# elucideye/acf

Measured on AMD Instinct MI355X. Metric: detector FPS @1080p, 8 scales/octave, FACE80 model, higher is better.
Workload: dtype f32

## Files before the change

### acf_amd/csrc/acf_hip.hip

```cpp
#include "kernels.hip.h"

#include <algorithm>
#include <cmath>
#include <cstdio>
#include <cstring>
#include <mutex>
#include <string>
#include <type_traits>
#include <vector>

using namespace acfhip;

namespace
{

struct DevBuf
{
    void* p = nullptr;
    size_t bytes = 0;
};

struct ResampleTiling
{
    int rows = 0, cols = 0, xo = 0, tile_y = 0, tile_x = 0;
// ... 108 lines not shown
    int tiles = 0, tileRows = 0, tileCols = 0;
    int maxCells = 0, maxBlocks = 0;
    float* d_tmp = nullptr;
    float* d_pyr = nullptr;
};

struct Options
{
    int taps = 0;
    int arith = 0;
    int profile = 0;
    int fusedSmooth = 1;
    int fusedGrad = 1;
    int fusedTri = 1;
    int sharedDevice = 0;
    int tilePersist = 1;
    int cascadeTiles = 1;
    int rankCells = 1;
    int scaleStreams = 1;
    int cascadeTurns = 0;
    int fusedLevels = 1;
    int smoothSegments = 0;
    int smoothWarm = 64, smoothForceRedo = 0;
    int levelSegments = 0;
    int levelWarm = 32;
    int countRepairs = 0;
    int keepPyramid = 1;
};

struct acf_hip_ctx
{
    int device = 0;
    hipStream_t stream = nullptr;
    bool ownStream = false;
    std::vector<hipStream_t> side;
    std::vector<acf_hip_ctx*> kids;
    int nStreams = 1, kidChunk = 0;
    hipEvent_t evFork = nullptr;
    std::vector<hipEvent_t> evJoin;
    mutable std::string err;
    bool hasModel = false, hasPlan = false;
    Options opt;
    bool x86Owned = false;
    uint32_t* d_x86 = nullptr;
    int numCus = 256;
    size_t ldsPerCu = size_t(160) * 1024;
    bool ranksValid = false;
    bool floatPyramid = true;
    std::vector<hipEvent_t> evPool;
    std::vector<const char*> evName;
    size_t evUsed = 0;
    std::vector<hipStream_t> evStream;
    std::vector<hipEvent_t> evScale;
    hipEvent_t evTurn[2] = { nullptr, nullptr };

    acf_hip_params p{};
    std::vector<uint32_t> fids, child;
    std::vector<float> thrs, hs;
    LdcfStage ldcf;

    Plan plan;
    bool autoLambdas = false;
    double* d_planeSums = nullptr;
    std::vector<double> h_lambdas;
    int maxBatch = 0, maxHits = 0, lastBatch = 0;
    bool pyramidValid = false, detectValid = false;

    std::vector<void*> allocs;
    float* d_lTable = nullptr;
    float* d_acos = nullptr;
    std::vector<RealScale> real;
    std::vector<ResampleDesc> h_descs;
    int nImgDescs = 0, nApproxDescs = 0;
    ResampleDesc* d_descs = nullptr;
    int32_t* d_it = nullptr;
    float* d_ft = nullptr;
    SmoothJob* d_realJobs = nullptr;
    SmoothJob* d_finalJobs = nullptr;
    LevelJob* d_levelJobs = nullptr;
    float* d_dump = nullptr;
    LevelJob* d_levelJobsRaw = nullptr;
    struct LevelGroup
    {
        int R, mode, first, count;
        double cost;
        int lane;
    };
    std::vector<LevelGroup> levelGroups, levelGroupsRaw;
    int nAllJobs = 0, nAllJobsRaw = 0;
    bool fusedOk = false;
    PadJob* d_padJobs = nullptr;
    PadJob* d_padJobsR = nullptr;
    bool levelsEmitRank = false;
    float *d_specState = nullptr, *d_trueState = nullptr;
    bool countersZeroed = false;
    int32_t* d_redo = nullptr;
    size_t redoInts = 0, lvRedoInts = 0;
    float *d_lvSpec = nullptr, *d_lvTrue = nullptr;
    int32_t* d_lvRedo = nullptr;
    int levelSegFrames = 0, levelSegCap = 0, levelHMax = 0;
    int useGraph = 0;
    struct GraphSlot
    {
        hipGraphExec_t exec = nullptr;
        const float* frames = nullptr;
        int n = 0;
// ... 46 lines not shown
    {
        int64_t chromaOff = 0, frameStride = 0;
    } yuv;
    uint8_t* d_yuvRgb = nullptr;
    size_t yuvRgbBytes = 0;
};

static inline bool rankCellsOn(const acf_hip_ctx* c, const CascState& cs)
{
    return cs.tilesR.ok && c->opt.rankCells;
}

#define HIPCHK(ctx, call)                                                                                  \
    do                                                                                                     \
    {                                                                                                      \
        hipError_t e_ = (call);                                                                            \
        if (e_ != hipSuccess)                                                                              \
        {                                                                                                  \
            (ctx)->err = std::string(#call) + ": " + hipGetErrorString(e_);                               \
            return ACF_HIP_E_HIP;                                                                          \
        }                                                                                                  \
    } while (0)

#define LAUNCHCHK(ctx, what)                                                                               \
    do                                                                                                     \
    {                                                                                                      \
        hipError_t e_ = hipGetLastError();                                                                 \
        if (e_ != hipSuccess)                                                                              \
        {                                                                                                  \
            (ctx)->err = std::string("launch ") + what + ": " + hipGetErrorString(e_);                    \
            return ACF_HIP_E_HIP;                                                                          \
        }                                                                                                  \
    } while (0)

namespace
{

enum : uint32_t
{
    FB_TRIY_UNFUSED = 1u << 0,
    FB_MOU_PLAIN = 1u << 1,
    FB_RESAMPLE_NO_STRIP = 1u << 2,
    FB_RESAMPLE_NO_PAIR = 1u << 3,
    FB_RESAMPLE_NO_UP = 1u << 4,
    FB_RESAMPLE_GENERIC = 1u << 5,
    FB_LEVEL_GROUPS = 1u << 6,
    FB_LDCF_UNFUSED = 1u << 7,
    FB_NO_DEDUP = 1u << 8,
    FB_NO_TAIL_CODES = 1u << 9,
    FB_TAIL3 = 1u << 10,
    FB_TILED_STAGED = 1u << 11,
    FB_TILED_POOLED1 = 1u << 12,
    FB_YUV_UNFUSED = 1u << 13,
};
uint32_t fallbackMask()
{
    static const uint32_t mask = [] {
        static const struct { const char* name; uint32_t bit; } kNames[] = {
            { "triy_unfused", FB_TRIY_UNFUSED }, { "mou_plain", FB_MOU_PLAIN }, { "resample_no_strip", FB_RESAMPLE_NO_STRIP },
            { "resample_no_pair", FB_RESAMPLE_NO_PAIR }, { "resample_no_up", FB_RESAMPLE_NO_UP }, { "resample_generic", FB_RESAMPLE_GENERIC },
            { "level_groups", FB_LEVEL_GROUPS }, { "ldcf_unfused", FB_LDCF_UNFUSED }, { "no_dedup", FB_NO_DEDUP }, { "no_tail_codes", FB_NO_TAIL_CODES },
            { "tail3", FB_TAIL3 }, { "tiled_staged", FB_TILED_STAGED }, { "tiled_pooled1", FB_TILED_POOLED1 },
            { "yuv_unfused", FB_YUV_UNFUSED } };
        uint32_t m = 0;
        const char* e = getenv("ACF_HIP_FORCE_FALLBACK");
        std::string s = e ? e : "";
        size_t i = 0;
        while (i < s.size())
        {
            size_t j = s.find(',', i);
            j = j == std::string::npos ? s.size() : j;
            const std::string tok = s.substr(i, j - i);
            bool known = tok.empty();
            for (const auto& n : kNames)
            {
                if (tok == n.name)
                {
                    m |= n.bit;
                    known = true;
                }
            }
            if (!known)
            {
                fprintf(stderr, "acf_hip: ACF_HIP_FORCE_FALLBACK: unknown name '%s'\n", tok.c_str());
                abort();
            }
            i = j + 1;
        }
        return m;
    }();
    return mask;
}
inline bool fallbackForced(uint32_t which)
{
    return (fallbackMask() & which) != 0;
}

int fail(const acf_hip_ctx* c, int code, const std::string& msg)
{
    c->err = msg;
    return code;
}

int needCtx(const acf_hip_ctx* c)
{
    return c ? ACF_HIP_OK : ACF_HIP_E_INVALID;
}
int needPlan(const acf_hip_ctx* c, const char* who, const char* hint = "")
{
    return !c ? ACF_HIP_E_INVALID : c->hasPlan ? ACF_HIP_OK : fail(c, ACF_HIP_E_NOPLAN, std::string(who) + ": plan first" + hint);
}
int needPlanRead(const acf_hip_ctx* c, const char* who)
{
    return c ? needPlan(c, who) : ACF_HIP_E_NOPLAN;
}
int needModel(const acf_hip_ctx* c, const char* who)
// ... 614 lines not shown
    {
        return ACF_HIP_OK;
    }
    std::lock_guard<std::mutex> lk(g_turnMu);
    HIPCHK(c, hipEventRecord(c->evTurn[which], c->stream));
    g_turnLast[chain][c->device] = c->evTurn[which];
    return ACF_HIP_OK;
}
void cascTurnForget(acf_hip_ctx* c)
{
    std::lock_guard<std::mutex> lk(g_turnMu);
    for (int w = 0; w < 2; w++)
    {
        if (c->evTurn[w])
        {
            for (int ch = 0; ch < 2; ch++)
            {
                if (c->device >= 0 && c->device < 64 && g_turnLast[ch][c->device] == c->evTurn[w])
                {
                    g_turnLast[ch][c->device] = nullptr;
                }
            }
            (void)hipEventDestroy(c->evTurn[w]);
            c->evTurn[w] = nullptr;
        }
    }
}
}

extern "C" {


int acf_hip_abi_version(void)
{
    return ACF_HIP_ABI_VERSION;
}

constexpr int ACF_SIDE_STREAMS = 6;
constexpr int LEVEL_MAX_R_REAL = 9;
static void ensureSide(acf_hip_ctx* c)
{
    while (int(c->side.size()) < std::min<int>(ACF_SIDE_STREAMS, int(c->evJoin.size())))
    {
        hipStream_t st;
        if (hipStreamCreateWithFlags(&st, hipStreamNonBlocking) != hipSuccess)
        {
            (void)hipGetLastError();
            break;
        }
        c->side.push_back(st);
    }
}

int acf_hip_create(int device, void* stream, acf_hip_ctx** out)
{
    if (!out)
    {
        return ACF_HIP_E_INVALID;
    }
    *out = nullptr;
    int n = 0;
    if (hipGetDeviceCount(&n) != hipSuccess || n <= 0 || device < 0 || device >= n)
    {
        return ACF_HIP_E_NODEVICE;
    }
    if (hipSetDevice(device) != hipSuccess)
    {
        return ACF_HIP_E_NODEVICE;
    }
    acf_hip_ctx* c = new (std::nothrow) acf_hip_ctx();
    if (!c)
    {
        return ACF_HIP_E_HIP;
    }
    c->device = device;
    {
        hipDeviceProp_t prop;
        if (hipGetDeviceProperties(&prop, device) == hipSuccess)
        {
            c->numCus = prop.multiProcessorCount > 0 ? prop.multiProcessorCount : c->numCus;
            c->ldsPerCu = prop.maxSharedMemoryPerMultiProcessor > 0 ? size_t(prop.maxSharedMemoryPerMultiProcessor) : c->ldsPerCu;
        }
    }
    if (stream)
    {
        c->stream = reinterpret_cast<hipStream_t>(stream);
    }
    else
    {
        if (hipStreamCreateWithFlags(&c->stream, hipStreamNonBlocking) != hipSuccess)
        {
            delete c;
            return ACF_HIP_E_HIP;
        }
        c->ownStream = true;
    }
    for (int i = 0; i < ACF_SIDE_STREAMS; i++)
    {
        hipEvent_t ev;
        if (hipEventCreateWithFlags(&ev, hipEventDisableTiming) == hipSuccess)
        {
            c->evJoin.push_back(ev);
        }
    }
    (void)hipEventCreateWithFlags(&c->evFork, hipEventDisableTiming);
    *out = c;
// ... 38 lines not shown
            if (!synced)
            {
                (void)hipSetDevice(c->device);
                (void)hipStreamSynchronize(c->stream);
                synced = true;
            }
            (void)hipGraphExecDestroy(g.exec);
        }
        g = acf_hip_ctx::GraphSlot();
    }
    c->graphNext = 0;
    c->plainRuns = 0;
}

int acf_hip_destroy(acf_hip_ctx* c)
{
    dropGraph(c);
    if (c)
    {
        for (acf_hip_ctx* k : c->kids)
        {
            (void)acf_hip_destroy(k);
        }
        c->kids.clear();
    }
    if (!c)
    {
        return ACF_HIP_E_INVALID;
    }
    (void)hipSetDevice(c->device);
    (void)hipStreamSynchronize(c->stream);
    (void)acf_hip_stream_close(c);
    cascTurnForget(c);
    freeAll(c);
    if (c->d_x86 && c->x86Owned)
    {
        (void)hipFree(c->d_x86);
    }
    for (hipEvent_t e : c->evPool)
    {
        (void)hipEventDestroy(e);
    }
    for (hipStream_t st : c->side)
    {
        (void)hipStreamDestroy(st);
    }
    for (hipEvent_t e : c->evJoin)
    {
        (void)hipEventDestroy(e);
    }
    if (c->evFork)
    {
        (void)hipEventDestroy(c->evFork);
    }
    for (hipEvent_t e : c->evScale)
    {
        (void)hipEventDestroy(e);
    }
    if (c->ownStream)
    {
        (void)hipStreamDestroy(c->stream);
    }
    delete c;
    return ACF_HIP_OK;
}

const char* acf_hip_last_error(const acf_hip_ctx* c)
{
    return c ? c->err.c_str() : "null context";
}

struct OptionKey
{
    const char* key;
    int Options::*field;
    bool nonzero;
    bool (*refuse)(const acf_hip_ctx*, int);
    const char* why;
    void (*after)(acf_hip_ctx*, int);
};

static bool negative(const acf_hip_ctx*, int v)
{
    return v < 0;
}

static const char* const LEVEL_RANGE = "option: level_warm a positive multiple of 4, level_segments >= 0";
static const char* const SMOOTH_RANGE = "option: smooth_segments >= 0, smooth_warm a multiple of 16";

static const OptionKey OPTION_KEYS[] = {
    { "graph", nullptr, false, nullptr, nullptr, [](acf_hip_ctx* c, int v) { c->useGraph = v; c->graphBroken = 0; } },
    { "streams", nullptr, false, [](const acf_hip_ctx*, int v) { return v < 1 || v > 6; }, "streams: 1..6",
        [](acf_hip_ctx* c, int v) { c->nStreams = v; } },
    { "taps", &Options::taps, true },
    { "arith", &Options::arith, true, [](const acf_hip_ctx* c, int v) { return v != 0 && !c->d_x86; },
        "arith: install a CPU's tables first (acf_hip_set_x86_tables)" },
    { "profile", &Options::profile, true, nullptr, nullptr, [](acf_hip_ctx* c, int) { c->evUsed = 0; } },
    { "fused_levels", &Options::fusedLevels, false },
    { "fused_smooth", &Options::fusedSmooth, true },
    { "fused_grad", &Options::fusedGrad, false },
    { "fused_tri", &Options::fusedTri, false },
    { "shared_device", &Options::sharedDevice, true },
    { "cascade_tiles", &Options::cascadeTiles, true },
    { "rank_cells", &Options::rankCells, true, nullptr, nullptr, [](acf_hip_ctx* c, int) { c->detectValid = false; } },
    { "tile_persist", &Options::tilePersist, false },
    { "cascade_turns", &Options::cascadeTurns, false },
// ... 1147 lines not shown
```

### acf_amd/csrc/kernels_channels.hip.h

```cpp
#pragma once

namespace acfhip
{

struct SmoothVecArgs
{
    const float* in;
    float* sm;
    float* half;
    float* chns;
    int64_t in_fs, in_ps, sm_fs, sm_ps, half_fs, half_ps, chns_fs, cells;
    int32_t h, w, plane0;
    float p, rkHalf, rq_y;
    float* dump;
    int32_t segW, warm, nSeg, nPlanes;
    int32_t segStride;
    float* specState;
    float* trueState;
    int32_t* redo;
    int32_t skipZ;
    float* gM;
    float* gO;
    const float* acos;
    int64_t mo_fs;
// ... 454 lines not shown
    {
        smooth_vec_body<true, HALF, true>(a, lds, z);
    }
    else
    {
        smooth_vec_body<false, HALF, true>(a, lds, z);
    }
}

template <bool HALF, bool ARITH = false>
__global__ void __launch_bounds__(64 * SV_MAXW) k_smooth_grad(SmoothVecArgs a, uint32_t fullMask)
{
    extern __shared__ float lds[];
    const int z = a.plane0;
    if (a.redo)
    {
        if (a.redo[int64_t(blockIdx.z) * a.nPlanes + z] == 0)
        {
            return;
        }
        __syncthreads();
        if (threadIdx.x == 0)
        {
            a.redo[int64_t(blockIdx.z) * a.nPlanes + z] = 0;
        }
    }
    float* acosL = lds + 2 * SV_MAXW * 2 * SV_K * 4;
    for (int i = threadIdx.x; i < GM_ACOS_N; i += blockDim.x)
    {
        acosL[i] = a.acos[i];
    }
    uint2* x86G = reinterpret_cast<uint2*>(acosL + GM_ACOS_N);
    float x86K = 0.f;
    if (ARITH)
    {
        const uint2* gsrc = reinterpret_cast<const uint2*>(a.x86 + X86_TABLE_N);
        for (int i = threadIdx.x; i < X86_GM_N; i += blockDim.x)
        {
            x86G[i] = gsrc[i];
        }
        x86K = __uint_as_float(a.x86[X86_TABLE_N + 2 * X86_GM_N]);
    }
    __syncthreads();
    if ((fullMask >> z) & 1u)
    {
        smooth_vec_body<true, HALF, true, true, false, ARITH>(a, lds, z, acosL + 10010, x86G, x86K);
    }
    else
    {
        smooth_vec_body<false, HALF, true, true, false, ARITH>(a, lds, z, acosL + 10010, x86G, x86K);
    }
}

template <bool HALF, bool ARITH = false>
__global__ void __launch_bounds__(512) k_smooth_grad_tri(SmoothVecArgs a, uint32_t fullMask)
{
    extern __shared__ float lds[];
    const int z = a.plane0;
    float* acosL = lds + 2 * SV_MAXW * 2 * SV_K * 4;
    for (int i = threadIdx.x; i < GM_ACOS_N; i += blockDim.x)
    {
        acosL[i] = a.acos[i];
    }
    uint2* x86G = reinterpret_cast<uint2*>(acosL + GM_ACOS_N);
    float x86K = 0.f;
    if (ARITH)
    {
        const uint2* gsrc = reinterpret_cast<const uint2*>(a.x86 + X86_TABLE_N);
        for (int i = threadIdx.x; i < X86_GM_N; i += blockDim.x)
        {
            x86G[i] = gsrc[i];
        }
        x86K = __uint_as_float(a.x86[X86_TABLE_N + 2 * X86_GM_N]);
    }
    __syncthreads();
    if ((fullMask >> z) & 1u)
    {
        smooth_vec_body<true, HALF, true, true, true, ARITH>(a, lds, z, acosL + 10010, x86G, x86K);
    }
    else
    {
        smooth_vec_body<false, HALF, true, true, true, ARITH>(a, lds, z, acosL + 10010, x86G, x86K);
    }
}

__global__ void __launch_bounds__(256) k_smooth_verify(const float* __restrict__ spec, const float* __restrict__ tru, int h, int segStride, int nPlanes,
    int32_t* __restrict__ redo, int force, int nSeg, int zG, int nSegG)
{
    const int64_t plane = int64_t(blockIdx.z) * nPlanes + blockIdx.y;
    const int s = 1 + blockIdx.x;
    if (s >= (int(blockIdx.y) == zG ? nSegG : nSeg))
    {
        return;
    }
    const uint32_t* a = reinterpret_cast<const uint32_t*>(spec) + (plane * segStride + s) * int64_t(h);
    const uint32_t* b = reinterpret_cast<const uint32_t*>(tru) + (plane * segStride + s) * int64_t(h);
    bool bad = force != 0;
    for (int y = threadIdx.x; y < h; y += 256)
    {
        bad = bad || (a[y] != b[y]);
    }
    if (bad)
    {
        redo[plane] = 1;
    }
}

struct SumJob
{
    int64_t off;
    int32_t cells;
    int32_t pad_;
};

__global__ void __launch_bounds__(256) k_plane_sums(const float* __restrict__ chns, int64_t chns_fs, SumJob j0, SumJob j1, int nPlanes, double* __restrict__ out)
{
    __shared__ double part[256];
    const int z = blockIdx.x, sel = blockIdx.y;
    const int64_t f = blockIdx.z;
    const SumJob J = sel ? j1 : j0;
    const float* __restrict__ src = chns + f * chns_fs + J.off + int64_t(z) * J.cells;
    double acc = 0.0;
    for (int i = threadIdx.x; i < J.cells; i += 256)
    {
        acc += double(src[i]);
    }
    part[threadIdx.x] = acc;
    __syncthreads();
    for (int s = 128; s >= 1; s >>= 1)
    {
        if (int(threadIdx.x) < s)
        {
            part[threadIdx.x] += part[threadIdx.x + s];
        }
        __syncthreads();
// ... 1231 lines not shown
```

### acf_amd/csrc/pyramid_run.hip.h

```cpp
#pragma once

namespace
{
struct ScalePlan
{
    bool fuseSm = false;
    bool halfNext = false;
    uint32_t fullMask = 0;
    bool wantGrad = false;
    bool triXFused = false;
    bool fuseCells = false;
    bool blocked = false;
    ChnsArgs a{};
    int nt = 0, warm = 0;
    int nSeg = 1, segW = 0;
    int nSegG = 1, segWG = 0;
    int segStride = 1;
    size_t ldsB = 0, ldsG = 0;
};

using SmoothVecKernel = void (*)(SmoothVecArgs, uint32_t);
using GradMagVecKernel = void (*)(const float*, float*, float*, const float*, int, int, int, int64_t, int64_t, int, int, const uint32_t*);
using LevelAllKernel = void (*)(const float*, float*, float*, const LevelJob*, const ResampleDesc*, const int32_t*, const float*, int, int64_t, int64_t, float,
    float*, int, LevelRankArgs, LevelSegArgs);
using LevelKernel = void (*)(const float*, float*, float*, const LevelJob*, const ResampleDesc*, const int32_t*, const float*, int, int64_t, int64_t, float,
    float*, int);

enum LevelsPath
{
    LV_FUSED,
    LV_WAVE_SMOOTH,
    LV_SMOOTH_JOBS,
    LV_COPY
};
struct LevelsCall
{
    LevelsPath path = LV_COPY;
    int nLF = 0;
    bool approxFirst = false;
    bool pad = false;
    float pS = 0.f;
    int64_t copyElems = 0;
    const LevelJob* jobs = nullptr;
    const std::vector<acf_hip_ctx::LevelGroup>* groups = nullptr;
    int nAll = 0;
    size_t nSide = 0;
    bool rawOut = false;
    bool emitRank = false, emitF32 = true;
    LevelRankArgs ra{};
    LevelSegArgs lsa{};
    size_t ldsL = 0;
    LevelAllKernel allKernel = nullptr;
    bool lvTurns = false;
    int lvChain = 1;
};

static SmoothVecKernel smoothGradKernel(bool tri, bool half, bool x86)
{
    if (!x86)
    {
        if (!tri)
        {
            return half ? k_smooth_grad<true, false> : k_smooth_grad<false, false>;
        }
        return half ? k_smooth_grad_tri<true, false> : k_smooth_grad_tri<false, false>;
    }
    if (!tri)
    {
        return half ? k_smooth_grad<true, true> : k_smooth_grad<false, true>;
    }
    return half ? k_smooth_grad_tri<true, true> : k_smooth_grad_tri<false, true>;
}

static SmoothVecKernel smoothVecKernel(bool half)
{
    return half ? k_smooth_vec<true> : k_smooth_vec<false>;
}

static GradMagVecKernel gradMagVecKernel(bool blocked, bool x86)
{
    if (blocked)
    {
        return x86 ? k_grad_mag_vec<true, true> : k_grad_mag_vec<true, false>;
    }
    return x86 ? k_grad_mag_vec<false, true> : k_grad_mag_vec<false, false>;
}

static LevelAllKernel levelAllKernel(bool f32, bool rank, bool segmented)
{
    if (f32 && rank)
    {
        return segmented ? k_level_all<LO_F32 | LO_RANK, 1> : k_level_all<LO_F32 | LO_RANK, 0>;
    }
    if (rank)
    {
        return segmented ? k_level_all<LO_RANK, 1> : k_level_all<LO_RANK, 0>;
    }
    return segmented ? k_level_all<LO_F32, 1> : k_level_all<LO_F32, 0>;
}

static LevelKernel levelKernel(int R, int mode)
{
#define LEVEL_R(RR)                                 \
    switch (mode)                                   \
    {                                               \
        case LM_REAL: return k_level<RR, LM_REAL>;  \
        case LM_DD: return k_level<RR, LM_DD>;      \
        default: return k_level<RR, LM_UU>;         \
    }
    switch (R)
    {
        case 1: LEVEL_R(1)
        case 2: LEVEL_R(2)
        case 3: LEVEL_R(3)
        case 4: LEVEL_R(4)
        case 5: LEVEL_R(5)
        case 6: LEVEL_R(6)
        case 7: LEVEL_R(7)
        case 8: LEVEL_R(8)
        default:
            return R == LEVEL_MAX_R_REAL && mode == LM_REAL ? k_level<9, LM_REAL> : nullptr;
    }
#undef LEVEL_R
}

static int countRepairs(acf_hip_ctx* c, hipStream_t st, const int32_t* d_flags, size_t n, int slot)
{
    if (!c->opt.countRepairs)
    {
        return ACF_HIP_OK;
    }
    std::vector<int32_t> fl(n);
    HIPCHK(c, hipMemcpyAsync(fl.data(), d_flags, n * 4, hipMemcpyDeviceToHost, st));
    HIPCHK(c, hipStreamSynchronize(st));
    c->repairs[slot] += int64_t(n);
    for (int32_t v : fl)
    {
        c->repairs[slot + 1] += v != 0;
    }
    return ACF_HIP_OK;
}

struct PyramidRun
{
    acf_hip_ctx* const c;
    const acf_hip_params& p;
    const Plan& pl;
    const int nF;
    const int H, W, d, d_in, shrink;
    const int64_t np0;
    const float* frames;
    const float* cur = nullptr;
    int64_t cur_fs = 0;
    int curH = 0, curW = 0;
    float pColor = 0.f;
    std::vector<int> srcIdx;
    std::vector<char> halfDone, pairDone;
    bool scalePar = false;
    hipStream_t st;
    LevelsCall lv;
    PackedSrc reduced{}, converted{};

    PyramidRun(acf_hip_ctx* ctx, const float* frames_, int nF_)
        : c(ctx), p(ctx->p), pl(ctx->plan), nF(nF_), H(pl.H), W(pl.W), d(pl.d), d_in(pl.d_in), shrink(ctx->p.shrink), np0(int64_t(pl.H) * pl.W), frames(frames_),
          st(ctx->stream)
    {
    }

    int ingest(const PackedSrc* u8, bool& ingestConverted);
    int colour(bool ingestConverted);
    int prepareScales();
    int realScale(size_t k);
    int imageResample(size_t k, const float*& img, int64_t& img_fs);
    ScalePlan planScale(size_t k, const float* img, int64_t img_fs);
    int smoothImage(size_t k, const float* img, int64_t img_fs, const ScalePlan& sp);
    int gradientChannels(size_t k, const ScalePlan& sp);
    int joinScales();
    int planLevels(int nLF);
    int levels(int f0, int nLF);
    int launchLevels(const LevelsCall& lc, int f0);
    int launchLevelAll(const LevelsCall& lc, int f0);
    int launchLevelGroups(const LevelsCall& lc, int f0);
    int padLevels(const LevelsCall& lc, int f0);
    int levelsWithImageLambdas();
};

int PyramidRun::ingest(const PackedSrc* u8, bool& ingestConverted)
{
    int rc;
    if (d_in == 5)
    {
        return fail(c, ACF_HIP_E_INVALID, "pyramid_u8: a plan for five input planes (image + M, O) takes float frames");
    }
    const int inRows = c->rz.on ? c->rz.rows : H, inCols = c->rz.on ? c->rz.cols : W;
    const bool fusedYuv = u8 && pixIsYuv(u8->pix) && !c->rz.on && !fallbackForced(FB_YUV_UNFUSED);
    if (u8 && pixIsYuv(u8->pix) && !fusedYuv)
    {
        U8Geom g;
        if (const char* bad = u8Geom(u8->pix, inRows, inCols, u8->rowStride, c->yuv.chromaOff, c->yuv.frameStride, g))
        {
            return fail(c, ACF_HIP_E_INVALID, std::string("pyramid_u8: ") + bad);
        }
        if (!u8PlanesOk(g, d_in))
        {
            return fail(c, ACF_HIP_E_INVALID, "pyramid_u8: the plan's input planes (d) must be 3 for NV12 / NV21");
        }
        const size_t need = size_t(c->maxBatch) * inRows * inCols * 3;
        if (c->yuvRgbBytes < need)
        {
            HIPCHK(c, hipStreamSynchronize(c->stream));
            devRelease(c, c->d_yuvRgb);
            c->yuvRgbBytes = 0;
            if ((rc = devAlloc(c, &c->d_yuvRgb, need)))
            {
                return rc;
            }
            c->yuvRgbBytes = need;
        }
        if ((rc = launchYuvToRgb(c, yuvSrc(u8->frames, u8->pix, inRows, inCols, g), nF, c->d_yuvRgb)))
        {
            return rc;
        }
        converted = PackedSrc{ c->d_yuvRgb, ACF_HIP_PIX_RGB, 0 };
        u8 = &converted;
    }
    if (u8 && c->rz.on)
    {
        U8Geom g;
// ... 69 lines not shown
        int curIdx = -1;
        for (size_t k = 0; k < c->real.size(); k++)
        {
            srcIdx[k] = curIdx;
            if (c->real[k].adoptAsI)
            {
                curIdx = int(k);
            }
        }
    }
    if (c->opt.scaleStreams && c->real.size() > 1 && !c->opt.taps)
    {
        ensureSide(c);
    }
    const size_t nSideS = c->side.size();
    scalePar = c->opt.scaleStreams && c->real.size() > 1 && nSideS >= c->real.size() - 1 && c->evJoin.size() >= nSideS && !c->opt.taps;
    while (scalePar && c->evScale.size() < c->real.size())
    {
        hipEvent_t e;
        HIPCHK(c, hipEventCreateWithFlags(&e, hipEventDisableTiming));
        c->evScale.push_back(e);
    }
    return ACF_HIP_OK;
}

int PyramidRun::realScale(size_t k)
{
    int rc;
    RealScale& rs = c->real[k];
    const int64_t np = int64_t(rs.h) * rs.w;
    if (scalePar)
    {
        if (k > 0)
        {
            prof(c, st, "(end)");
        }
        st = k == 0 ? c->stream : c->side[k - 1];
        if (k > 0)
        {
            HIPCHK(c, hipStreamWaitEvent(st, c->evScale[k - 1], 0));
        }
    }
    const float* img = cur;
    int64_t img_fs = cur_fs;
    if (rs.resampled && (rc = imageResample(k, img, img_fs)))
    {
        return rc;
    }
    const ScalePlan sp = planScale(k, img, img_fs);
    if ((rc = smoothImage(k, img, img_fs, sp)))
    {
        return rc;
    }
    if (scalePar)
    {
        HIPCHK(c, hipEventRecord(c->evScale[k], st));
    }
    if (rs.adoptAsI)
    {
        cur = rs.sm;
        cur_fs = int64_t(d) * np;
        curH = rs.h;
        curW = rs.w;
    }
    return gradientChannels(k, sp);
}

int PyramidRun::imageResample(size_t k, const float*& img, int64_t& img_fs)
{
    RealScale& rs = c->real[k];
    const int64_t np = int64_t(rs.h) * rs.w;
    if (rs.src_h != curH || rs.src_w != curW)
    {
        return fail(c, ACF_HIP_E_INVALID, "pyramid: internal plan mismatch");
    }
    if (c->h_descs[rs.descIndex].src_frame_stride != cur_fs)
    {
        return fail(c, ACF_HIP_E_INVALID, "pyramid: internal frame-stride mismatch");
    }
    prof(c, st, "k_resample(image)");
    const ResampleDesc& hd = c->h_descs[rs.descIndex];
    const bool exactHalf = hd.xmode == RS_EXACT && hd.ymode == RS_EXACT && hd.xk == 2 && hd.yk == 2 && hd.ha % 4 == 0 && hd.hb % 2 == 0 &&
        hd.src_frame_stride % 4 == 0 && hd.dst_frame_stride % 2 == 0 && hd.src_off % 4 == 0 && hd.dst_off % 2 == 0 &&
        (uintptr_t(cur) & 15) == 0 && (uintptr_t(rs.img) & 7) == 0;
    if (halfDone[k] || pairDone[k])
    {
    }
    else if (rs.strip.ok && !exactHalf && !resampleGenericOnly() && (uintptr_t(cur) & 15) == 0)
    {
        const bool pair = rs.stripPair.ok && k + 1 < c->real.size() && srcIdx[k + 1] == srcIdx[k] && !c->opt.taps && !scalePar;
        if (pair)
        {
            pairDone[k + 1] = 1;
        }
        launchStrip(c, st, pair ? rs.stripPair : rs.strip, c->d_descs, rs.descIndex, pair ? c->real[k + 1].descIndex : -1, hd.nplanes, cur, rs.img,
            pair ? c->real[k + 1].img : nullptr, c->d_it, c->d_ft, nF);
    }
    else if (exactHalf)
    {
        const int64_t items = int64_t(hd.hb / 2) * hd.wb * hd.nplanes;
        hipLaunchKernelGGL(k_resample_half, dim3(cdiv(items, 256), 1, nF), dim3(256), 0, st, cur, rs.img,
            (const ResampleDesc*)(c->d_descs + rs.descIndex));
    }
    else if (resampleUpOk(hd) && !resampleGenericOnly() && (uintptr_t(rs.img) & 15) == 0)
    {
        const int nw = hd.nplanes * cdiv(hd.hb, 256) * cdiv(hd.wb, RSU_XC);
        hipLaunchKernelGGL(k_resample_up, dim3(cdiv(nw, 4), 1, nF), dim3(256), 0, st, cur, rs.img,
            (const ResampleDesc*)(c->d_descs + rs.descIndex), (const int32_t*)c->d_it, (const float*)c->d_ft);
    }
    else
    {
        const int xt = int64_t(resampleBlocks(hd)) * nF < 4096 ? 2 : RS_XT;
        hipLaunchKernelGGL(k_resample, dim3(resampleBlocks(hd, xt), 1, nF), dim3(64, 4), 0, st, cur, rs.img,
            (const ResampleDesc*)(c->d_descs + rs.descIndex), (const int32_t*)c->d_it, (const float*)c->d_ft, xt);
    }
    LAUNCHCHK(c, "k_resample(image)");
    img = rs.img;
    img_fs = int64_t(d) * np;
// ... 9 lines not shown
    ScalePlan sp;
    sp.fuseSm = p.colorSmooth > 0 && p.colorEnabled && !c->opt.taps && c->opt.fusedSmooth && shrink == 4 && rs.h % 4 == 0 && rs.w % 4 == 0 && rs.w >= 16 &&
        rs.h / 4 <= SV_MAXW * SV_OWN && img_fs % 4 == 0 && np % 4 == 0 && (uintptr_t(img) & 15) == 0;
    ChnsArgs& a = sp.a;
    a.sm = rs.sm;
    a.M = rs.M;
    a.S = rs.S;
    a.O = rs.O;
    a.Mn = c->opt.taps ? rs.Mn : nullptr;
    a.chns = c->d_chns + pl.raw_off[rs.level];
    a.sm_fs = int64_t(d) * np;
    a.m_fs = np;
    a.chns_fs = pl.raw_floats;
    a.h = rs.h;
    a.w = rs.w;
    a.d = d;
    a.colorEnabled = p.colorEnabled;
    a.colorDone = sp.fuseSm ? 1 : 0;
    a.magEnabled = p.gradMagEnabled;
    a.histEnabled = p.gradHistEnabled;
    a.nOrients = p.nOrients;
    a.doNorm = p.normRad != 0;
    a.full = p.full;
    a.hardBin = p.softBin < 0;
    a.normConst = float(p.normConst);
    a.rq_y = shrinkGainY(shrink);
    const bool gradVec = rs.h % 4 == 0 && np % 4 == 0;
    sp.fuseCells = shrink == 4 && !c->opt.taps;
    sp.blocked = grad && p.normRad && !moWithImage &&
        triPlan(rs.M, rs.U, rs.h, rs.w, p.normRad, np, sp.fuseCells ? &a : nullptr, rs.uFloats, rs.moFloats, gradVec).blocked;
    if (!sp.fuseSm)
    {
        return sp;
    }
    sp.halfNext = k + 1 < c->real.size() && srcIdx[k + 1] == int(k) && c->real[k + 1].resampled && [&] {
        const ResampleDesc& nd = c->h_descs[c->real[k + 1].descIndex];
        return nd.xmode == RS_EXACT && nd.ymode == RS_EXACT && nd.xk == 2 && nd.yk == 2 && nd.ha == rs.h && nd.wa == rs.w;
    }();
    bool needFullAll = false;
    for (size_t m = k + 1; m < c->real.size(); m++)
    {
        if (srcIdx[m] == int(k) && !(m == k + 1 && sp.halfNext))
        {
            needFullAll = true;
        }
    }
    sp.nt = cdiv(rs.h / 4, SV_OWN) * 64;
    const int64_t gradMinPx = int64_t(1) << 20;
    const int gradMinF = 16;
    sp.wantGrad = grad && gradVec && !moWithImage && (c->opt.fusedGrad >= 2 || (c->opt.fusedGrad == 1 && np >= gradMinPx && nF >= gradMinF));
    const int triMinF = 64;
    sp.triXFused = sp.wantGrad && sp.blocked && p.normRad == 5 && rs.w >= 48 && sp.nt <= 512 &&
        (c->opt.fusedTri >= 2 || (c->opt.fusedTri == 1 && c->opt.sharedDevice && nF >= triMinF));
    for (int z = 0; z < d; z++)
    {
        if (needFullAll || (grad && z == p.colorChn && !sp.wantGrad))
        {
            sp.fullMask |= 1u << z;
        }
    }
    sp.warm = std::max(16, c->opt.smoothWarm);
    auto segmentsFor = [&](int planesOf, int& segW_) {
        int n = c->opt.smoothSegments;
        if (n == 0 && c->opt.sharedDevice && nF >= 64)
        {
            n = 1;
        }
        if (n == 0)
        {
            const int64_t waves = int64_t(std::max(planesOf, 1)) * nF * (sp.nt / 64);
            n = int(std::min<int64_t>((6 * 1024 + waves - 1) / waves, rs.w / (4 * sp.warm)));
        }
        n = std::max(1, std::min(n, std::min(c->segCap, rs.w / 16)));
        segW_ = cdiv(cdiv(rs.w, n), 16) * 16;
        return cdiv(rs.w, segW_);
    };
    if (!sp.wantGrad)
    {
        sp.nSeg = sp.nSegG = segmentsFor(d, sp.segW);
        sp.segWG = sp.segW;
    }
    else
    {
        if (sp.triXFused)
        {
            sp.nSegG = 1;
            sp.segWG = cdiv(rs.w, 16) * 16;
        }
        else
        {
            sp.nSegG = segmentsFor(1, sp.segWG);
        }
        sp.nSeg = sp.nSegG;
        sp.segW = sp.segWG;
        if (d > 1)
        {
            sp.nSeg = segmentsFor(d - 1, sp.segW);
        }
    }
    sp.segStride = std::max(sp.nSeg, sp.nSegG);
    sp.ldsB = size_t(2) * SV_MAXW * 2 * SV_K * 4 * sizeof(float);
    sp.ldsG = sp.ldsB + size_t(GM_ACOS_N) * sizeof(float) + (c->opt.arith ? size_t(X86_GM_N) * sizeof(uint2) : 0);
    return sp;
}

int PyramidRun::smoothImage(size_t k, const float* img, int64_t img_fs, const ScalePlan& sp)
{
    int rc;
    RealScale& rs = c->real[k];
    const int64_t np = int64_t(rs.h) * rs.w;
    if (!sp.fuseSm)
    {
        if (p.colorSmooth > 0)
        {
            return launchSmooth(c, st, img, rs.sm, c->d_realJobs + k, 1, d, rs.h, img_fs, int64_t(d) * np, nF, pColor, true);
        }
        hipLaunchKernelGGL(k_copy_planes, dim3(cdiv(np * d, 256), 1, nF), dim3(256), 0, st, img, rs.sm, (const SmoothJob*)(c->d_realJobs + k), img_fs,
            int64_t(d) * np);
        LAUNCHCHK(c, "k_copy_planes");
        return ACF_HIP_OK;
    }
    SmoothVecArgs sa{};
    sa.in = img;
    sa.in_fs = img_fs;
    sa.in_ps = np;
    sa.sm = rs.sm;
    sa.sm_fs = int64_t(d) * np;
    sa.sm_ps = np;
    sa.chns = c->d_chns + pl.raw_off[rs.level];
    sa.chns_fs = pl.raw_floats;
    sa.cells = int64_t(rs.h / 4) * (rs.w / 4);
    sa.h = rs.h;
    sa.w = rs.w;
    sa.p = pColor;
    sa.rq_y = shrinkGainY(shrink);
    sa.dump = c->d_dump;
    if (sp.halfNext)
    {
        const RealScale& nx = c->real[k + 1];
        sa.half = nx.img;
        sa.half_ps = int64_t(nx.h) * nx.w;
        sa.half_fs = int64_t(d) * sa.half_ps;
        sa.rkHalf = c->h_descs[nx.descIndex].rk[0];
        halfDone[k + 1] = true;
    }
    sa.plane0 = 0;
    sa.nPlanes = d;
    sa.segW = sp.segW;
    sa.warm = sp.warm;
    sa.nSeg = sp.nSeg;
    sa.segStride = sp.segStride;
    sa.specState = c->d_specState;
    sa.trueState = c->d_trueState;
    sa.redo = nullptr;
    sa.skipZ = -1;
    if (sp.wantGrad)
    {
        sa.skipZ = p.colorChn;
        sa.gM = rs.M;
        sa.gO = rs.O;
        sa.acos = c->d_acos;
        sa.mo_fs = sp.blocked ? moBlockedFloats(rs.h, rs.w) : np;
        sa.nybM = sp.blocked ? (rs.h + 15) / 16 : 0;
        sa.full = p.full;
        if (sp.triXFused)
        {
            sa.tU = rs.U;
            sa.u_fs = uBlockedFloats(rs.h, rs.w);
            sa.nybU = (rs.h + 8 + 15) / 16;
        }
    }
    auto gradArgs = [&](int segW, int nSeg) {
        SmoothVecArgs g = sa;
        g.plane0 = p.colorChn;
        g.skipZ = -1;
        g.segW = segW;
        g.nSeg = nSeg;
        g.x86 = x86T(c);
        return g;
    };
    const SmoothVecKernel gradKernel = smoothGradKernel(sp.triXFused, sp.halfNext, x86T(c) != nullptr), vecKernel = smoothVecKernel(sp.halfNext);
    const char* gradName = sp.triXFused ? "k_smooth_grad_tri" : "k_smooth_grad";
    const int nVec = sp.wantGrad ? d - 1 : d;
    if (sp.wantGrad)
    {
        if ((rc = allowLds(c, reinterpret_cast<const void*>(gradKernel), sp.ldsG)))
        {
            return rc;
        }
        prof(c, st, gradName);
        hipLaunchKernelGGL(gradKernel, dim3(1, sp.nSegG, nF), dim3(sp.nt), sp.ldsG, st, gradArgs(sp.segWG, sp.nSegG), sp.fullMask);
    }
    if (nVec > 0)
    {
        prof(c, st, "k_smooth_vec");
        hipLaunchKernelGGL(vecKernel, dim3(nVec, sp.nSeg, nF), dim3(sp.nt), sp.ldsB, st, sa, sp.fullMask);
    }
    LAUNCHCHK(c, "k_smooth_vec");
    if (sp.segStride == 1)
    {
        return ACF_HIP_OK;
    }
    hipLaunchKernelGGL(k_smooth_verify, dim3(sp.segStride - 1, d, nF), dim3(256), 0, st, (const float*)c->d_specState, (const float*)c->d_trueState,
        rs.h, sp.segStride, d, c->d_redo, c->opt.smoothForceRedo, sp.nSeg, sp.wantGrad ? p.colorChn : -1, sp.nSegG);
    LAUNCHCHK(c, "k_smooth_verify");
    if ((rc = countRepairs(c, st, c->d_redo, size_t(nF) * d, 0)))
    {
        return rc;
    }
    sa.segW = rs.w;
    sa.warm = 0;
    sa.nSeg = 1;
    sa.redo = c->d_redo;
    if (sp.wantGrad)
    {
        prof(c, st, gradName);
        if (sp.nSegG > 1)
        {
            hipLaunchKernelGGL(gradKernel, dim3(1, 1, nF), dim3(sp.nt), sp.ldsG, st, gradArgs(rs.w, 1), sp.fullMask);
        }
    }
    if (nVec > 0)
    {
        prof(c, st, "k_smooth_vec");
        hipLaunchKernelGGL(vecKernel, dim3(nVec, 1, nF), dim3(sp.nt), sp.ldsB, st, sa, sp.fullMask);
    }
    LAUNCHCHK(c, "k_smooth_vec(repair)");
    return ACF_HIP_OK;
}

int PyramidRun::gradientChannels(size_t k, const ScalePlan& sp)
{
    int rc;
    RealScale& rs = c->real[k];
    const int64_t np = int64_t(rs.h) * rs.w;
    ChnsArgs a = sp.a;
    if (d_in == 5 && k == 0)
    {
        a.M = frames + 3 * np0;
        a.O = frames + 4 * np0;
        a.S = nullptr;
        a.Mn = nullptr;
        a.m_fs = int64_t(d_in) * np0;
        a.doNorm = 0;
        return launchChns(c, st, a, shrink, nF);
    }
    a.x86 = x86T(c);
    if ((p.gradMagEnabled || p.gradHistEnabled) && !sp.wantGrad)
    {
        prof(c, st, "k_grad_mag");
        if (rs.h % 4 == 0 && np % 4 == 0)
        {
            const int64_t items = int64_t(cdiv(rs.w, GMV_XT)) * (rs.h / 4) * nF;
            const int gmvMax = 256;
            const int blocks = int(std::min<int64_t>(gmvMax, (items + GMV_BLOCK - 1) / GMV_BLOCK));
            hipLaunchKernelGGL(gradMagVecKernel(sp.blocked, a.x86 != nullptr), dim3(blocks), dim3(GMV_BLOCK), 0, st,
                (const float*)(rs.sm + int64_t(p.colorChn) * np), rs.M, rs.O, (const float*)c->d_acos, rs.h, rs.w, p.full, int64_t(d) * np,
                sp.blocked ? moBlockedFloats(rs.h, rs.w) : np, nF, sp.blocked ? (rs.h + 15) / 16 : 0, a.x86);
        }
        else
        {
            const int rowBlocks = cdiv(rs.h, GM_ROWS), nStrips = cdiv(rs.w, GM_XT);
            const int want = std::max(1, cdiv(1024, rowBlocks * nF));
            const int spb = std::max(8, cdiv(nStrips, want));
            hipLaunchKernelGGL(k_grad_mag_strip, dim3(rowBlocks, cdiv(nStrips, spb), nF), dim3(GM_ROWS), 0, st,
                (const float*)(rs.sm + int64_t(p.colorChn) * np), rs.M, rs.O, (const float*)c->d_acos, rs.h, rs.w, p.full, int64_t(d) * np, np, spb, x86T(c));
        }
        LAUNCHCHK(c, "k_grad_mag");
    }
    bool cellsDone = false;
    if ((p.gradMagEnabled || p.gradHistEnabled) && p.normRad)
    {
        if ((rc = launchTri(c, st, rs.M, rs.U, rs.S, rs.h, rs.w, p.normRad, np, nF, sp.fuseCells ? &a : nullptr, &cellsDone, rs.uFloats, rs.moFloats,
                 sp.blocked, sp.triXFused)))
        {
            return rc;
        }
    }
    return cellsDone ? ACF_HIP_OK : launchChns(c, st, a, shrink, nF);
}
// ... 272 lines not shown
    }
    HIPCHK(c, hipStreamSynchronize(st));
    return ACF_HIP_OK;
}

int pyramidBody(acf_hip_ctx* c, const float* frames, const PackedSrc* u8, int nF)
{
    if (c && !c->kids.empty())
    {
        if (u8)
        {
            return fail(c, ACF_HIP_E_UNSUPPORTED, "pyramid_u8: not available with option \"streams\" > 1");
        }
        if (!frames || nF <= 0 || nF > c->maxBatch)
        {
            return fail(c, ACF_HIP_E_INVALID, "pyramid: n_frames out of range");
        }
        const size_t per = size_t(c->plan.d_in) * c->plan.H * c->plan.W;
        const int rc = forEachKid(c, nF, [&](acf_hip_ctx* k, int first, int n) { return acf_hip_pyramid(k, frames + first * per, n); });
        if (!rc)
        {
            c->lastBatch = nF;
            c->pyramidValid = true;
            c->detectValid = false;
        }
        return rc;
    }
    if (int rc = needPlan(c, "pyramid")) return rc;
    if ((!frames && !u8) || (u8 && !u8->frames) || nF <= 0 || nF > c->maxBatch)
    {
        return fail(c, ACF_HIP_E_INVALID, "pyramid: n_frames out of range");
    }
    HIPCHK(c, hipSetDevice(c->device));
    c->pyramidValid = c->detectValid = false;
    int rc;
    PyramidRun run(c, frames, nF);
    bool ingestConverted = false;
    if (u8 && (rc = run.ingest(u8, ingestConverted)))
    {
        return rc;
    }
    c->lastFrames = run.frames;
    if ((rc = run.colour(ingestConverted)) || (rc = run.prepareScales()))
    {
        return rc;
    }
    for (size_t k = 0; k < c->real.size(); k++)
    {
        if ((rc = run.realScale(k)))
        {
            return rc;
        }
    }
    if ((rc = run.joinScales()))
    {
        return rc;
    }
    if (!c->autoLambdas)
    {
        for (int f = 0; f < nF; f++)
        {
            c->h_lambdas[size_t(f) * 3 + 0] = c->p.lambdas[0];
            c->h_lambdas[size_t(f) * 3 + 1] = c->p.lambdas[1];
            c->h_lambdas[size_t(f) * 3 + 2] = c->p.lambdas[2];
        }
        if ((rc = run.levels(0, nF)))
        {
            return rc;
        }
    }
    else if ((rc = run.levelsWithImageLambdas()))
    {
        return rc;
    }
    prof(c, c->stream, "(end)");
    c->lastBatch = nF;
    c->pyramidValid = true;
    c->ranksValid = run.lv.emitRank;
    c->floatPyramid = run.lv.emitF32;
    return ACF_HIP_OK;
}
}
```

Baseline: 16470.

## Run scale-0 gradient kernel on a side stream beside smoothing and later scales

For the full-resolution scale, the gradient/triangle kernel is split out of the fused smoothing launch. It runs without cell output, as one unsegmented launch on a side stream (or a device-shared chain stream), while the vector smoothing covers all channels. Scale 0's gradient channels are deferred until after the other scales are queued, so the gradient chain can overlap with downstream resampling. This adds event syncs, a global mutex and extra smoothing work for the colour channel. The single-segment gradient launch may also lose parallelism.

```diff
diff --git a/acf_amd/csrc/acf_hip.hip b/acf_amd/csrc/acf_hip.hip
--- a/acf_amd/csrc/acf_hip.hip
+++ b/acf_amd/csrc/acf_hip.hip
@@ -184,6 +184,7 @@
     size_t evUsed = 0;
     std::vector<hipStream_t> evStream;
     std::vector<hipEvent_t> evScale;
+    hipEvent_t evChain[2] = { nullptr, nullptr };
     hipEvent_t evTurn[2] = { nullptr, nullptr };
 
     acf_hip_params p{};
@@ -336,6 +337,7 @@
     FB_TILED_STAGED = 1u << 11,
     FB_TILED_POOLED1 = 1u << 12,
     FB_YUV_UNFUSED = 1u << 13,
+    FB_GRAD_INLINE = 1u << 14,
 };
 uint32_t fallbackMask()
 {
@@ -345,7 +347,7 @@
             { "resample_no_pair", FB_RESAMPLE_NO_PAIR }, { "resample_no_up", FB_RESAMPLE_NO_UP }, { "resample_generic", FB_RESAMPLE_GENERIC },
             { "level_groups", FB_LEVEL_GROUPS }, { "ldcf_unfused", FB_LDCF_UNFUSED }, { "no_dedup", FB_NO_DEDUP }, { "no_tail_codes", FB_NO_TAIL_CODES },
             { "tail3", FB_TAIL3 }, { "tiled_staged", FB_TILED_STAGED }, { "tiled_pooled1", FB_TILED_POOLED1 },
-            { "yuv_unfused", FB_YUV_UNFUSED } };
+            { "yuv_unfused", FB_YUV_UNFUSED }, { "grad_inline", FB_GRAD_INLINE } };
         uint32_t m = 0;
         const char* e = getenv("ACF_HIP_FORCE_FALLBACK");
         std::string s = e ? e : "";
@@ -1066,6 +1068,40 @@
     }
 }
 
+static std::mutex g_chainMu;
+static hipStream_t g_chainStream[64] = {};
+static int chainStream(acf_hip_ctx* c, hipStream_t* out, bool* shared)
+{
+    hipStreamCaptureStatus cap = hipStreamCaptureStatusNone;
+    HIPCHK(c, hipStreamIsCapturing(c->stream, &cap));
+    *shared = c->opt.sharedDevice && cap == hipStreamCaptureStatusNone && c->device >= 0 && c->device < 64;
+    for (hipEvent_t& e : c->evChain)
+    {
+        if (!e)
+        {
+            HIPCHK(c, hipEventCreateWithFlags(&e, hipEventDisableTiming));
+        }
+    }
+    if (*shared)
+    {
+        std::lock_guard<std::mutex> lk(g_chainMu);
+        hipStream_t& st = g_chainStream[c->device];
+        if (!st)
+        {
+            HIPCHK(c, hipStreamCreateWithFlags(&st, hipStreamNonBlocking));
+        }
+        *out = st;
+        return ACF_HIP_OK;
+    }
+    ensureSide(c);
+    if (c->side.empty())
+    {
+        return fail(c, ACF_HIP_E_HIP, "pyramid: no side stream for the gradient chain");
+    }
+    *out = c->side[0];
+    return ACF_HIP_OK;
+}
+
 int acf_hip_create(int device, void* stream, acf_hip_ctx** out)
 {
     if (!out)
@@ -1210,6 +1246,13 @@
     if (c->evFork)
     {
         (void)hipEventDestroy(c->evFork);
+    }
+    for (hipEvent_t e : c->evChain)
+    {
+        if (e)
+        {
+            (void)hipEventDestroy(e);
+        }
     }
     for (hipEvent_t e : c->evScale)
     {
diff --git a/acf_amd/csrc/kernels_channels.hip.h b/acf_amd/csrc/kernels_channels.hip.h
--- a/acf_amd/csrc/kernels_channels.hip.h
+++ b/acf_amd/csrc/kernels_channels.hip.h
@@ -530,7 +530,7 @@
     }
 }
 
-template <bool HALF, bool ARITH = false>
+template <bool HALF, bool ARITH = false, bool CELLS = true>
 __global__ void __launch_bounds__(512) k_smooth_grad_tri(SmoothVecArgs a, uint32_t fullMask)
 {
     extern __shared__ float lds[];
@@ -554,11 +554,11 @@
     __syncthreads();
     if ((fullMask >> z) & 1u)
     {
-        smooth_vec_body<true, HALF, true, true, true, ARITH>(a, lds, z, acosL + 10010, x86G, x86K);
+        smooth_vec_body<true, HALF, CELLS, true, true, ARITH>(a, lds, z, acosL + 10010, x86G, x86K);
     }
     else
     {
-        smooth_vec_body<false, HALF, true, true, true, ARITH>(a, lds, z, acosL + 10010, x86G, x86K);
+        smooth_vec_body<false, HALF, CELLS, true, true, ARITH>(a, lds, z, acosL + 10010, x86G, x86K);
     }
 }
 
diff --git a/acf_amd/csrc/pyramid_run.hip.h b/acf_amd/csrc/pyramid_run.hip.h
--- a/acf_amd/csrc/pyramid_run.hip.h
+++ b/acf_amd/csrc/pyramid_run.hip.h
@@ -9,6 +9,7 @@
     uint32_t fullMask = 0;
     bool wantGrad = false;
     bool triXFused = false;
+    bool gradBeside = false;
     bool fuseCells = false;
     bool blocked = false;
     ChnsArgs a{};
@@ -55,8 +56,12 @@
     int lvChain = 1;
 };
 
-static SmoothVecKernel smoothGradKernel(bool tri, bool half, bool x86)
-{
+static SmoothVecKernel smoothGradKernel(bool tri, bool half, bool x86, bool cells = true)
+{
+    if (!cells)
+    {
+        return x86 ? k_smooth_grad_tri<false, true, false> : k_smooth_grad_tri<false, false, false>;
+    }
     if (!x86)
     {
         if (!tri)
@@ -159,6 +164,8 @@
     bool scalePar = false;
     hipStream_t st;
     LevelsCall lv;
+    ScalePlan sp0;
+    bool chainPending = false;
     PackedSrc reduced{}, converted{};
 
     PyramidRun(acf_hip_ctx* ctx, const float* frames_, int nF_)
@@ -174,6 +181,8 @@
     int imageResample(size_t k, const float*& img, int64_t& img_fs);
     ScalePlan planScale(size_t k, const float* img, int64_t img_fs);
     int smoothImage(size_t k, const float* img, int64_t img_fs, const ScalePlan& sp);
+    int gradChain(const SmoothVecArgs& g, const ScalePlan& sp);
+    int finishScale0();
     int gradientChannels(size_t k, const ScalePlan& sp);
     int joinScales();
     int planLevels(int nLF);
@@ -349,7 +358,7 @@
     {
         return rc;
     }
-    if (scalePar)
+    if (scalePar && !sp.gradBeside)
     {
         HIPCHK(c, hipEventRecord(c->evScale[k], st));
     }
@@ -360,7 +369,23 @@
         curH = rs.h;
         curW = rs.w;
     }
+    if (k == 0 && chainPending)
+    {
+        sp0 = sp;
+        return ACF_HIP_OK;
+    }
     return gradientChannels(k, sp);
+}
+
+int PyramidRun::finishScale0()
+{
+    if (!chainPending)
+    {
+        return ACF_HIP_OK;
+    }
+    chainPending = false;
+    HIPCHK(c, hipStreamWaitEvent(st, c->evChain[1], 0));
+    return gradientChannels(0, sp0);
 }
 
 int PyramidRun::imageResample(size_t k, const float*& img, int64_t& img_fs)
@@ -476,6 +501,7 @@
     const int triMinF = 64;
     sp.triXFused = sp.wantGrad && sp.blocked && p.normRad == 5 && rs.w >= 48 && sp.nt <= 512 &&
         (c->opt.fusedTri >= 2 || (c->opt.fusedTri == 1 && c->opt.sharedDevice && nF >= triMinF));
+    sp.gradBeside = k == 0 && sp.triXFused && sp.halfNext && !fallbackForced(FB_GRAD_INLINE);
     for (int z = 0; z < d; z++)
     {
         if (needFullAll || (grad && z == p.colorChn && !sp.wantGrad))
@@ -517,9 +543,9 @@
         }
         sp.nSeg = sp.nSegG;
         sp.segW = sp.segWG;
-        if (d > 1)
-        {
-            sp.nSeg = segmentsFor(d - 1, sp.segW);
+        if (sp.gradBeside || d > 1)
+        {
+            sp.nSeg = segmentsFor(sp.gradBeside ? d : d - 1, sp.segW);
         }
     }
     sp.segStride = std::max(sp.nSeg, sp.nSegG);
@@ -580,7 +606,7 @@
     sa.skipZ = -1;
     if (sp.wantGrad)
     {
-        sa.skipZ = p.colorChn;
+        sa.skipZ = sp.gradBeside ? -1 : p.colorChn;
         sa.gM = rs.M;
         sa.gO = rs.O;
         sa.acos = c->d_acos;
@@ -605,8 +631,15 @@
     };
     const SmoothVecKernel gradKernel = smoothGradKernel(sp.triXFused, sp.halfNext, x86T(c) != nullptr), vecKernel = smoothVecKernel(sp.halfNext);
     const char* gradName = sp.triXFused ? "k_smooth_grad_tri" : "k_smooth_grad";
-    const int nVec = sp.wantGrad ? d - 1 : d;
-    if (sp.wantGrad)
+    const int nVec = sp.wantGrad && !sp.gradBeside ? d - 1 : d;
+    if (sp.gradBeside)
+    {
+        if (!scalePar && (rc = gradChain(gradArgs(sp.segWG, 1), sp)))
+        {
+            return rc;
+        }
+    }
+    else if (sp.wantGrad)
     {
         if ((rc = allowLds(c, reinterpret_cast<const void*>(gradKernel), sp.ldsG)))
         {
@@ -621,12 +654,20 @@
         hipLaunchKernelGGL(vecKernel, dim3(nVec, sp.nSeg, nF), dim3(sp.nt), sp.ldsB, st, sa, sp.fullMask);
     }
     LAUNCHCHK(c, "k_smooth_vec");
+    auto chainBehind = [&]() -> int {
+        if (!sp.gradBeside || !scalePar)
+        {
+            return ACF_HIP_OK;
+        }
+        HIPCHK(c, hipEventRecord(c->evScale[k], st));
+        return gradChain(gradArgs(sp.segWG, 1), sp);
+    };
     if (sp.segStride == 1)
     {
-        return ACF_HIP_OK;
+        return chainBehind();
     }
     hipLaunchKernelGGL(k_smooth_verify, dim3(sp.segStride - 1, d, nF), dim3(256), 0, st, (const float*)c->d_specState, (const float*)c->d_trueState,
-        rs.h, sp.segStride, d, c->d_redo, c->opt.smoothForceRedo, sp.nSeg, sp.wantGrad ? p.colorChn : -1, sp.nSegG);
+        rs.h, sp.segStride, d, c->d_redo, c->opt.smoothForceRedo, sp.nSeg, sp.wantGrad && !sp.gradBeside ? p.colorChn : -1, sp.nSegG);
     LAUNCHCHK(c, "k_smooth_verify");
     if ((rc = countRepairs(c, st, c->d_redo, size_t(nF) * d, 0)))
     {
@@ -636,7 +677,7 @@
     sa.warm = 0;
     sa.nSeg = 1;
     sa.redo = c->d_redo;
-    if (sp.wantGrad)
+    if (sp.wantGrad && !sp.gradBeside)
     {
         prof(c, st, gradName);
         if (sp.nSegG > 1)
@@ -650,6 +691,42 @@
         hipLaunchKernelGGL(vecKernel, dim3(nVec, 1, nF), dim3(sp.nt), sp.ldsB, st, sa, sp.fullMask);
     }
     LAUNCHCHK(c, "k_smooth_vec(repair)");
+    return chainBehind();
+}
+
+int PyramidRun::gradChain(const SmoothVecArgs& g, const ScalePlan& sp)
+{
+    int rc;
+    const SmoothVecKernel kernel = smoothGradKernel(true, false, g.x86 != nullptr, false);
+    if ((rc = allowLds(c, reinterpret_cast<const void*>(kernel), sp.ldsG)))
+    {
+        return rc;
+    }
+    hipStream_t cst = st;
+    bool shared = false;
+    if (!scalePar && (rc = chainStream(c, &cst, &shared)))
+    {
+        return rc;
+    }
+    std::unique_lock<std::mutex> lk(g_chainMu, std::defer_lock);
+    if (shared)
+    {
+        lk.lock();
+    }
+    if (!scalePar)
+    {
+        HIPCHK(c, hipEventRecord(c->evChain[0], st));
+        HIPCHK(c, hipStreamWaitEvent(cst, c->evChain[0], 0));
+    }
+    prof(c, cst, "k_smooth_grad_tri");
+    hipLaunchKernelGGL(kernel, dim3(1, 1, nF), dim3(sp.nt), sp.ldsG, cst, g, sp.fullMask & ~(1u << p.colorChn));
+    LAUNCHCHK(c, "k_smooth_grad_tri");
+    if (!scalePar)
+    {
+        prof(c, cst, "(end)");
+        HIPCHK(c, hipEventRecord(c->evChain[1], cst));
+        chainPending = true;
+    }
     return ACF_HIP_OK;
 }
 
@@ -1028,7 +1105,7 @@
             return rc;
         }
     }
-    if ((rc = run.joinScales()))
+    if ((rc = run.finishScale0()) || (rc = run.joinScales()))
     {
         return rc;
     }
```

Result: slower. 15020 (-8.8%).
